# iamarkaj/AwesomeSLAM

Measured on AMD Instinct MI355X. Metric: EKF/UKF filter-steps/s @ N_landmarks, higher is better.
Workload: dtype f32

## Files before the change

awesomeslam_amd/core.py:

```python
import ctypes
import os
import subprocess

import numpy as np

_CSRC = os.path.join(os.path.dirname(os.path.abspath(__file__)), "csrc")
_CORE = os.path.join(_CSRC, "libaslam_core.so")
_NODE = os.path.join(_CSRC, "libaslam_node.so")

EKF, UKF = 0, 1
F64, F32 = 0, 1
FILTERS = {"ekf": EKF, "ukf": UKF}

ST_GROWTH_REFUSED, ST_WAIT_OVERFLOW, ST_NOT_PD, ST_OBS_OVERFLOW, ST_INTERNAL = 1, 2, 4, 8, 16
CFG_UKF_LARGE = 1

CORE_SYMBOLS = (
    "aslam_create", "aslam_destroy", "aslam_reset", "aslam_last_error", "aslam_abi_version", "aslam_set_state",
    "aslam_grow", "aslam_ekf_step", "aslam_ukf_step", "aslam_ekf_step_batch", "aslam_ukf_step_batch", "aslam_set_trace", "aslam_replay", "aslam_get_dim",
    "aslam_get_state", "aslam_get_A", "aslam_get_landmarks", "aslam_get_wait", "aslam_get_status",
    "aslam_get_layout", "aslam_kernel_info", "aslam_get_launch_info",
    "aslam_replay_stats", "aslam_innovation_enable", "aslam_get_innovation",
    "aslam_params_default", "aslam_set_params", "aslam_get_params",
    "aslam_remove_landmarks", "aslam_select_beyond",
    "aslam_get_sightings", "aslam_select_stale",
    "aslam_sighted_update_enable", "aslam_get_sighted", "aslam_ekf_step_sighted", "aslam_ekf_step_batch_sighted",
)
NODE_SYMBOLS = (
    "aslam_node_create", "aslam_node_create_at", "aslam_node_destroy", "aslam_node_error", "aslam_node_sensor", "aslam_node_odom",
    "aslam_node_odom_now", "aslam_node_dim", "aslam_node_get", "aslam_node_wait", "aslam_node_core",
    "aslam_host_narrow_odom", "aslam_node_enable_innovation", "aslam_node_innovation",
    "aslam_node_set_params", "aslam_node_get_params", "aslam_node_remove_landmarks",
    "aslam_node_get_sightings", "aslam_node_remove_stale", "aslam_node_set_sighted_only",
)
TRACE_FILE_SYMBOLS = (
    "aslam_trace_file_open", "aslam_trace_file_close", "aslam_trace_file_error", "aslam_trace_file_dims",
    "aslam_trace_file_view", "aslam_trace_file_raw", "aslam_trace_file_write",
)


class AslamError(RuntimeError):
    pass


class Config(ctypes.Structure):
    _fields_ = [(k, ctypes.c_int32) for k in
                ("filter", "dtype", "max_landmark_count", "batch", "max_obs", "max_wait", "device", "flags")]


class TraceView(ctypes.Structure):
    _fields_ = [("T", ctypes.c_int64), ("max_obs", ctypes.c_int32), ("is_device", ctypes.c_int32),
                ("pose", ctypes.c_void_p), ("yaw", ctypes.c_void_p), ("twist", ctypes.c_void_p),
                ("dt", ctypes.c_void_p), ("obs_new", ctypes.c_void_p), ("n_obs", ctypes.c_void_p),
                ("obs", ctypes.c_void_p)]
# ... 80 lines not shown
                          "(there is no CPU fallback for the filter core)")
        import torch

        L = ctypes.CDLL(_CORE)
        vp, ci, cf, cd = ctypes.c_void_p, ctypes.c_int, ctypes.c_float, ctypes.c_double
        pd, pf, pi, pu = (ctypes.POINTER(t) for t in (ctypes.c_double, ctypes.c_float, ctypes.c_int, ctypes.c_uint32))
        L.aslam_last_error.restype = ctypes.c_char_p
        L.aslam_create.argtypes = [ctypes.POINTER(Config), ctypes.POINTER(vp)]
        L.aslam_destroy.argtypes = [vp]
        L.aslam_reset.argtypes = [vp]
        L.aslam_set_state.argtypes = [vp, ci, ci, pd, pd, pd]
        L.aslam_grow.argtypes = [vp, ci, ci, pd, pd]
        L.aslam_ekf_step.argtypes = [vp, ci, cf, cf, cf, pd, cd, cd, pd, vp]
        L.aslam_ukf_step.argtypes = [vp, ci, cf, cf, cf, pd, pd, vp]
        L.aslam_ekf_step_batch.argtypes = [vp, pf, pf, pf, pd, ci, pd, pd, pd, ci, vp]
        L.aslam_ukf_step_batch.argtypes = [vp, pf, pf, pf, pd, ci, pd, ci, vp]
        L.aslam_set_trace.argtypes = [vp, ctypes.POINTER(TraceView)]
        L.aslam_replay.argtypes = [vp, ctypes.c_int64, ctypes.c_int64, vp, vp, vp]
        L.aslam_replay_stats.argtypes = [vp, ctypes.c_int64, ctypes.c_int64, vp, vp, vp, vp, vp, vp]
        L.aslam_innovation_enable.argtypes = [vp, ci]
        L.aslam_get_innovation.argtypes = [vp, ci, pd, pd]
        L.aslam_params_default.argtypes = [ctypes.POINTER(Params)]
        L.aslam_set_params.argtypes = [vp, ci, ctypes.POINTER(Params)]
        L.aslam_get_params.argtypes = [vp, ci, ctypes.POINTER(Params)]
        L.aslam_get_dim.argtypes = [vp, ci, pi]
        L.aslam_get_state.argtypes = [vp, ci, pd, pd, pd]
        L.aslam_get_A.argtypes = [vp, ci, pd, pd]
        L.aslam_get_landmarks.argtypes = [vp, ci, pd, pd, pi]
        L.aslam_get_wait.argtypes = [vp, ci, pf, pf, pu, ci, pi]
        L.aslam_get_status.argtypes = [vp, ci, pu]
        L.aslam_get_layout.argtypes = [vp, pi, ctypes.POINTER(ctypes.c_int64)]
        L.aslam_kernel_info.argtypes = [vp, ctypes.c_char_p, ci, pi, pi, pi]
        L.aslam_get_launch_info.argtypes = [vp, pi, pi, pi]
        L.aslam_remove_landmarks.argtypes = [vp, vp, ci, ci, vp]
        L.aslam_select_beyond.argtypes = [vp, pd, vp, ci, vp]
        L.aslam_get_sightings.argtypes = [vp, ci, pu, pu, ci, pi, pu]
        L.aslam_select_stale.argtypes = [vp, pu, vp, ci, vp]
        pb = ctypes.POINTER(ctypes.c_uint8)
        L.aslam_sighted_update_enable.argtypes = [vp, ci]
        L.aslam_get_sighted.argtypes = [vp, ci, pb, ci, pi]
        L.aslam_ekf_step_sighted.argtypes = [vp, ci, cf, cf, cf, pd, pb, cd, cd, pd, vp]
        L.aslam_ekf_step_batch_sighted.argtypes = [vp, pf, pf, pf, pd, ci, pb, ci, pd, pd, pd, ci, vp]
        p32, p64 = ctypes.POINTER(ctypes.c_int32), ctypes.POINTER(ctypes.c_int64)
        L.aslam_snapshot_record_bytes.restype = ctypes.c_int64
        L.aslam_snapshot_record_bytes.argtypes = [ci, ci, ci]
        L.aslam_snapshot_check.argtypes = [vp, ctypes.c_int64, p32, p32]
        L.aslam_snapshot.argtypes = [vp, p32, ci, vp, ctypes.c_int64, ci, p64, vp]
        L.aslam_restore.argtypes = [vp, p32, p32, ci, vp, ctypes.c_int64, ci, vp]
        _core = L
    return _core


def node_lib():
    global _node
    if _node is None:
        if not os.path.exists(_NODE):
            raise OSError(f"{_NODE} is missing: run __graft_entry__.build()")
        core_lib()
        L = ctypes.CDLL(_NODE)
        vp, ci = ctypes.c_void_p, ctypes.c_int
        pd, pf, pu = (ctypes.POINTER(t) for t in (ctypes.c_double, ctypes.c_float, ctypes.c_uint32))
        L.aslam_node_create.restype = vp
        L.aslam_node_create.argtypes = [ci, ci, ci]
        L.aslam_node_create_at.restype = vp
        L.aslam_node_create_at.argtypes = [ci, ci, ci, ctypes.c_double]
        L.aslam_node_destroy.argtypes = [vp]
# ... 422 lines not shown
        return (before - after) // 2

    def replay_forget(self, t0, nsteps, period, max_age, poses_ptr=None, dims_ptr=None, stream=None):
        t0, nsteps, period = int(t0), int(nsteps), int(period)
        if period < 1:
            raise ValueError("period must be at least 1")
        mask, ld = self._device_mask()
        dims, done = [], 0
        while done < nsteps:
            k = min(period, nsteps - done)
            self.replay(t0 + done, k, None if poses_ptr is None else poses_ptr + 8 * 3 * self.batch * done,
                        None if dims_ptr is None else dims_ptr + 4 * self.batch * done, stream)
            self.select_stale(max_age, mask.data_ptr(), ld, stream)
            dims.append(self.remove_landmarks(mask, stream=stream))
            done += k
        return np.array(dims, np.int64).reshape(len(dims), self.batch)

    def layout(self):
        npad, nbytes = ctypes.c_int(), ctypes.c_int64()
        _chk(core_lib().aslam_get_layout(self._h, ctypes.byref(npad), ctypes.byref(nbytes)))
        return npad.value, nbytes.value

    def kernel_info(self):
        name = ctypes.create_string_buffer(192)
        g, b, l = ctypes.c_int(), ctypes.c_int(), ctypes.c_int()
        _chk(core_lib().aslam_kernel_info(self._h, name, 192, ctypes.byref(g), ctypes.byref(b), ctypes.byref(l)))
        return {"name": name.value.decode(), "grid": g.value, "block": b.value, "lds_bytes": l.value}

    def launch_info(self):
        g, r, l = ctypes.c_int(), ctypes.c_int(), ctypes.c_int()
        _chk(core_lib().aslam_get_launch_info(self._h, ctypes.byref(g), ctypes.byref(r), ctypes.byref(l)))
        return {"stream_groups": g.value, "chol_resident": bool(r.value), "launches_per_callback": l.value}


class Node:

    def __init__(self, filter="ekf", max_landmark_count=30, device=0, now_init=0.0):
        h = node_lib().aslam_node_create_at(FILTERS[filter], int(max_landmark_count), int(device), float(now_init))
        if not h:
            raise AslamError(node_lib().aslam_node_error().decode())
        self._h = ctypes.c_void_p(h)

    def close(self):
        if getattr(self, "_h", None):
            node_lib().aslam_node_destroy(self._h)
            self._h = None

    __del__ = close

    def sensor_msg(self, xs, ys):
        xs = np.ascontiguousarray(xs, np.float64)
        ys = np.ascontiguousarray(ys, np.float64)
        node_lib().aslam_node_sensor(self._h, len(xs), _ptr(xs, ctypes.c_double), _ptr(ys, ctypes.c_double))

    def odom_msg(self, msg8, dt):
        m = np.ascontiguousarray(msg8, np.float64)
        rc = node_lib().aslam_node_odom(self._h, _ptr(m, ctypes.c_double), float(np.float32(dt)))
        if rc < 0:
            raise AslamError(node_lib().aslam_node_error().decode())
        return rc

    def odom_msg_now(self, msg8, now):
        m = np.ascontiguousarray(msg8, np.float64)
        rc = node_lib().aslam_node_odom_now(self._h, _ptr(m, ctypes.c_double), float(now))
        if rc < 0:
            raise AslamError(node_lib().aslam_node_error().decode())
# ... 82 lines not shown
```

awesomeslam_amd/csrc/aslam_core.hip:

```cpp
#include "../../include/aslam_core.h"
#include "../../include/aslam_scan.h"
#include "../../include/aslam_snapshot.h"

#include <hip/hip_runtime.h>

#include <cmath>
#include <cstdio>
#include <cstring>
#include <cstdlib>
#include <algorithm>
#include <mutex>
#include <string>
#include <type_traits>
#include <vector>

#include "ekf_small.h"
#include "ekf_large.h"
#include "ekf_large_launch.h"
#include "scan_front.h"
#include "snapshot.h"
#include "prune.h"
#if ASLAM_HAVE_UKF
#include "ukf_small.h"
#include "ukf_large.h"
// ... 1616 lines not shown
                hipLaunchKernelGGL(scan_landmarks_kernel, dim3((unsigned)count), dim3(64), 0, st, d_in, tab, tab + SCAN_BEAMS, count, max_out, d_r,
                                   d_b, d_n, d_s);
                e = hipGetLastError();
        }
        if (e == hipSuccess)
                e = hipMemcpyAsync(range_out, d_r, n * max_out * sizeof(float), hipMemcpyDeviceToHost, st);
        if (e == hipSuccess)
                e = hipMemcpyAsync(bearing_out, d_b, n * max_out * sizeof(float), hipMemcpyDeviceToHost, st);
        if (e == hipSuccess)
                e = hipMemcpyAsync(n_out, d_n, n * sizeof(int32_t), hipMemcpyDeviceToHost, st);
        if (e == hipSuccess)
                e = hipMemcpyAsync(status_out, d_s, n * sizeof(uint32_t), hipMemcpyDeviceToHost, st);
        if (e == hipSuccess)
                e = hipStreamSynchronize(st);
        cleanup();
        if (e != hipSuccess)
                return fail(ASLAM_ERR_HIP, std::string("aslam_scan_landmarks: ") + hipGetErrorString(e));
        return ASLAM_OK;
}

int aslam_get_launch_info(aslam_ctx *c, int *stream_groups, int *chol_resident, int *launches_per_callback)
{
        if (!c)
                return fail(ASLAM_ERR_ARG, "null context");
        if (stream_groups)
                *stream_groups = c->large ? c->lh.last_groups : 0;
        if (chol_resident)
                *chol_resident = c->large && c->lh.last_resident;
        if (launches_per_callback)
                *launches_per_callback = c->large ? c->lh.last_launches : 1;
        return ASLAM_OK;
}

int aslam_kernel_info(aslam_ctx *c, char *name, int name_cap, int *grid, int *block, int *lds_bytes)
{
        if (!c)
                return fail(ASLAM_ERR_ARG, "null context");
        char buf[192];
        size_t lds = 0;
        if (c->large)
        {
                const LargePlan plan = large_plan(c->cfg.dtype == ASLAM_F32, c->NP, c->cfg.batch, c->cfg.batch, c->lh.knobs);
#if ASLAM_HAVE_UKF
                if (c->cfg.filter == ASLAM_UKF)
                        std::snprintf(buf, sizeof(buf), "ukf_large_wabt + large_update_panel<double> + large_syrk<double> (%d-launch chain per callback, 1 stream)",
                                      ukf_large_plan(c->NP).launches);
                else
#endif
                if (plan.chain == LargeChain::F32_RESIDENT)
                        std::snprintf(buf, sizeof(buf), "%s + %s + large_syrk_bf16x3%s (%d-launch chain per callback, %d stream groups)",
                                      plan.chol16 ? "large_chol_bf16" : "large_chol_resident", plan.trsm16 ? "large_trsm_bf16" : "large_trsm_pipe<17>",
                                      plan.border ? " + border" : "", plan.launches, c->lh.knobs.groups);
                else if (plan.chain == LargeChain::F32_RIGHT)
                        std::snprintf(buf, sizeof(buf), "large_right_step + large_syrk_bf16x3 (%d-launch chain per callback: one right-looking launch per block column)", plan.launches);
                else if (plan.chain == LargeChain::F32_LEFT)
                        std::snprintf(buf, sizeof(buf), "large_trsm_pipe<17> + large_syrk_bf16x3 (%d-launch chain per callback: multi-workgroup Cholesky)", plan.launches);
                else
                        std::snprintf(buf, sizeof(buf), "large_update_panel<double> (%d-launch chain per callback, %d stream groups)", plan.launches, c->lh.knobs.groups);
                lds = LargeLds::bytes(c->NP);
                if (c->sighted_on && c->cfg.filter == ASLAM_EKF)
                {
                        const std::string with = std::string("large_build_GS<T,sighted> + ") + buf;
                        std::snprintf(buf, sizeof(buf), "%s", with.c_str());
                }
        }
        else if (c->cfg.filter == ASLAM_EKF)
// ... 27 lines not shown
```

awesomeslam_amd/csrc/ekf_large.h:

```cpp
#pragma once

#include <type_traits>

#include "small_common.h"

namespace aslam
{
constexpr int LB = 64;
constexpr int LARGE_OBS_CAP = 1024;
constexpr int LARGE_WAIT_CAP = 2048;
constexpr int LARGE_NP_MAX = 1088;
constexpr int LARGE_NB_MAX = LARGE_NP_MAX / LB;

template <typename T> struct LargeView
{
        int NP;
        double *P;
        T *G;
        T *S;
        double *Hc;
        double *Y;
        T *Linv;
        T *Vw;
        unsigned short *Lpl;
        int xrows;
        int border;
};

typedef float f4 __attribute__((ext_vector_type(4)));
template <typename T> struct Mfma;
template <> struct Mfma<double>
{
        typedef d4 acc_t;
        static __device__ __forceinline__ acc_t zero()
        {
                return (acc_t){0.0, 0.0, 0.0, 0.0};
        }
        static __device__ __forceinline__ acc_t mma(double a, double b, acc_t c)
        {
                return __builtin_amdgcn_mfma_f64_16x16x4f64(a, b, c, 0, 0, 0);
        }
        static __device__ __forceinline__ int row(int lane, int r)
        {
                return (lane >> 4) + 4 * r;
        }
};
template <> struct Mfma<float>
{
        typedef f4 acc_t;
        static __device__ __forceinline__ acc_t zero()
        {
                return (acc_t){0.f, 0.f, 0.f, 0.f};
        }
        static __device__ __forceinline__ acc_t mma(float a, float b, acc_t c)
        {
                return __builtin_amdgcn_mfma_f32_16x16x4f32(a, b, c, 0, 0, 0);
        }
        static __device__ __forceinline__ int row(int lane, int r)
        {
// ... 31 lines not shown
        const size_t np = (size_t)v.NP;
        f(v.P, np * np, false);
        f(v.G, np * np, true);
        f(v.S, np * np, true);
        f(v.Hc, (np / 2) * 4, false);
        f(v.Y, np, false);
        f(v.Linv, (size_t)LARGE_NB_MAX * LB * LB, false);
        f(v.Lpl, LPlanes::per_filter(v.NP), false);
        f(v.Vw, np * np, true);
}

__host__ __device__ __forceinline__ int lplane_pos(int c)
{
        return 32 * (c >> 5) + 8 * ((c >> 2) & 3) + 4 * ((c >> 4) & 1) + (c & 3);
}

__host__ __device__ __forceinline__ int large_blocks(int n, int xrows = 1)
{
        return (n + xrows + LB - 1) / LB;
}

struct LargeBorder
{
        int t;
        int nbc;
};
__host__ __device__ __forceinline__ LargeBorder large_border(int n, int enabled)
{
        const int n0 = n & ~(LB - 1), t = n - n0;
        const bool on = enabled && n0 >= LB && (t == 1 || t == 3);
        return {on ? t : 0, on ? n0 / LB : large_blocks(n)};
}
constexpr int BORDER_MAX = 3;
constexpr int BORDER_SAVE = 8, BORDER_SAVE_ROWS = 4;
__host__ __device__ __forceinline__ bool border_spare(const LargeBorder &bd, int n, int row, int col)
{
        return bd.t && row > n && row <= n + bd.t && (col < LB * bd.nbc || (col >= LB * bd.nbc + BORDER_SAVE && col < LB * bd.nbc + BORDER_SAVE + BORDER_SAVE_ROWS));
}

struct LargeLds
{
        static __host__ __device__ size_t bytes(int NP)
        {
                size_t o = 0;
                o += 8 * (size_t)NP * 2;
                o += 4 * (size_t)LARGE_OBS_CAP * 6;
                o += 4 * (size_t)LARGE_WAIT_CAP * 5;
                o += 4 * (size_t)(NP / 2);
                o += 4 * (size_t)LARGE_OBS_CAP * 4 * 2;
                o += 4 * (size_t)NP;
                o = (o + 15) & ~(size_t)15;
                return o + sizeof(SmallShared);
        }
        static __device__ __forceinline__ SmallLds carve(unsigned char *smem, int NP)
        {
                SmallLds L;
                unsigned char *p = smem;
                L.Lt = nullptr;
                L.Dinv = nullptr;
                L.sY = nullptr;
                L.sU = nullptr;
                L.sH = nullptr;
                L.sTv = nullptr;
                L.sX = reinterpret_cast<double *>(p);
                p += 8 * (size_t)NP;
                L.sZ = reinterpret_cast<double *>(p);
// ... 887 lines not shown
constexpr int XU_WAVES = ASLAM_XU_WAVES;
constexpr int XU_THREADS = 64 * XU_WAVES;
constexpr int XU_WG_ROWS = XU_WAVES * XU_ROWS;
typedef double xu_d2 __attribute__((ext_vector_type(2)));
constexpr int XU_STAGE_THREADS = 256;
static_assert(XU_WAVES >= 4 && XU_WAVES <= 16, "large_x_update_rows: 4 staging waves at least, 1024 threads at most");

template <bool RUNNING>
__global__ __launch_bounds__(256, 3) void large_syrk_bf16x3(DevView d, LargeView<float> lv, int nfilters, const int *skipped)
{
        constexpr int TB = 128, KC = 32;
        constexpr int LDB = KC;
        typedef __bf16 bf8 __attribute__((ext_vector_type(8)));
        typedef unsigned u4 __attribute__((ext_vector_type(4)));
        typedef unsigned u2 __attribute__((ext_vector_type(2)));
        __shared__ __attribute__((aligned(16))) unsigned short As[3][TB * LDB];
        __shared__ __attribute__((aligned(16))) unsigned short Bs[3][TB * LDB];
        const int ntile = (lv.NP + TB - 1) / TB, nlow = ntile * (ntile + 1) / 2;
        const int slot = blockIdx.x >> 3;
        const int b = (slot / nlow) * 8 + (blockIdx.x & 7);
        if (b >= nfilters || skipped[b])
                return;
        const int n = d.n[b], NP = lv.NP;
        const int na = large_blocks(n) * LB;
        const int tl = slot % nlow;
        int rt = (int)((sqrtf(8.0f * (float)tl + 1.0f) - 1.0f) * 0.5f);
        while ((rt + 1) * (rt + 2) / 2 <= tl)
                ++rt;
        while (rt * (rt + 1) / 2 > tl)
                --rt;
        const int jt = tl - rt * (rt + 1) / 2;
        if (rt * TB >= n)
                return;
        const int tid = threadIdx.x, wave = tid >> 6, lane = tid & 63, li = lane & 15, lg = lane >> 4;
        const int wr = (wave >> 1) * 64, wc = (wave & 1) * 64;
        const float *G = lv.G + (size_t)b * NP * NP;
        double *P = lv.P + (size_t)b * NP * NP;
        constexpr int LPR = KC / 4, RPP = 256 / LPR, NPASS = TB / RPP;
        const int lrow = tid / LPR, lc0 = (tid % LPR) * 4;
        const float *Ap[NPASS], *Bp[NPASS];
#pragma unroll
        for (int q = 0; q < NPASS; ++q)
        {
                Ap[q] = G + (size_t)min(rt * TB + lrow + RPP * q, na - 1) * NP + lc0;
                Bp[q] = G + (size_t)min(jt * TB + lrow + RPP * q, na - 1) * NP + lc0;
        }
        f4 acc[4][4];
#pragma unroll
        for (int u = 0; u < 4; ++u)
#pragma unroll
                for (int v = 0; v < 4; ++v)
                        acc[u][v] = (f4){0.f, 0.f, 0.f, 0.f};
        f4 ta[NPASS], tb[NPASS];
        auto fetch = [&](int kc) {
#pragma unroll
                for (int q = 0; q < NPASS; ++q)
                {
                        ta[q] = *reinterpret_cast<const f4 *>(Ap[q] + kc);
                        tb[q] = *reinterpret_cast<const f4 *>(Bp[q] + kc);
                }
        };
        typedef float f2 __attribute__((ext_vector_type(2)));
        typedef __bf16 bf2 __attribute__((ext_vector_type(2)));
        auto stash = [&](unsigned short (&S)[3][TB * LDB], int off, const f4 &x) {
                unsigned pk[3][2];
#pragma unroll
                for (int e = 0; e < 2; ++e)
                {
                        const f2 v = {x[2 * e], x[2 * e + 1]};
                        const bf2 h = __builtin_convertvector(v, bf2);
                        const f2 r1 = v - __builtin_convertvector(h, f2);
                        const bf2 m = __builtin_convertvector(r1, bf2);
                        const f2 r2 = r1 - __builtin_convertvector(m, f2);
                        const bf2 l = __builtin_convertvector(r2, bf2);
                        pk[0][e] = __builtin_bit_cast(unsigned, h), pk[1][e] = __builtin_bit_cast(unsigned, m), pk[2][e] = __builtin_bit_cast(unsigned, l);
                }
#pragma unroll
                for (int p = 0; p < 3; ++p)
                        *reinterpret_cast<u2 *>(&S[p][off]) = (u2){pk[p][0], pk[p][1]};
        };
        const bool idle = (rt == jt && wc > wr);
        const bool diagq = (rt == jt && wc == wr);
        const int nu = idle ? 0 : __builtin_amdgcn_readfirstlane(max(0, min(4, (n - (rt * TB + wr) + 15) >> 4)));
        const int nv = idle ? 0 : __builtin_amdgcn_readfirstlane(max(0, min(4, (n - (jt * TB + wc) + 15) >> 4)));
        const bool full = !RUNNING && nu == 4 && nv == 4 && !diagq;
        const int kend = min(na, (n + KC - 1) / KC * KC);
        const int a_off = (wr + li) * LDB + 8 * (lg ^ (li >> 2)), b_off = (wc + li) * LDB + 8 * (lg ^ (li >> 2));
        const int s_off = lrow * LDB + 8 * ((lc0 >> 3) ^ ((lrow & 15) >> 2)) + (lc0 & 4);
        fetch(0);
        for (int kc = 0; kc < kend; kc += KC)
        {
#pragma unroll
                for (int q = 0; q < NPASS; ++q)
                {
                        stash(As, s_off + RPP * q * LDB, ta[q]);
                        stash(Bs, s_off + RPP * q * LDB, tb[q]);
                }
                __syncthreads();
                if (kc + KC < kend)
                        fetch(kc + KC);
#define ASLAM_MM(t, bb, aa, c) t = __builtin_amdgcn_mfma_f32_16x16x32_bf16(__builtin_bit_cast(bf8, bb), __builtin_bit_cast(bf8, aa), c, 0, 0, 0)
                if (full)
                {
#pragma unroll
                        for (int vh = 0; vh < 4; vh += 2)
                        {
                                u4 bq[2][3];
#pragma unroll
                                for (int v = 0; v < 2; ++v)
#pragma unroll
                                        for (int p = 0; p < 3; ++p)
                                                bq[v][p] = *reinterpret_cast<const u4 *>(&Bs[p][b_off + 16 * (vh + v) * LDB]);
                                f4 pa = {0.f, 0.f, 0.f, 0.f}, pb = {0.f, 0.f, 0.f, 0.f};
#pragma unroll
                                for (int u = 0; u < 4; ++u)
                                {
                                        u4 ap[3];
#pragma unroll
                                        for (int p = 0; p < 3; ++p)
                                                ap[p] = *reinterpret_cast<const u4 *>(&As[p][a_off + 16 * u * LDB]);
                                        f4 ta, tb;
                                        ASLAM_MM(ta, bq[0][0], ap[2], ((f4){0.f, 0.f, 0.f, 0.f}));
                                        ASLAM_MM(tb, bq[1][0], ap[2], ((f4){0.f, 0.f, 0.f, 0.f}));
                                        ASLAM_MM(ta, bq[0][1], ap[1], ta);
                                        ASLAM_MM(tb, bq[1][1], ap[1], tb);
                                        ASLAM_MM(ta, bq[0][2], ap[0], ta);
                                        ASLAM_MM(tb, bq[1][2], ap[0], tb);
                                        if (u > 0)
                                        {
                                                acc[u - 1][vh] += pa;
                                                acc[u - 1][vh + 1] += pb;
                                        }
                                        ASLAM_MM(ta, bq[0][0], ap[1], ta);
                                        ASLAM_MM(tb, bq[1][0], ap[1], tb);
                                        ASLAM_MM(ta, bq[0][1], ap[0], ta);
                                        ASLAM_MM(tb, bq[1][1], ap[0], tb);
                                        ASLAM_MM(ta, bq[0][0], ap[0], ta);
                                        ASLAM_MM(tb, bq[1][0], ap[0], tb);
                                        pa = ta, pb = tb;
                                        __builtin_amdgcn_sched_barrier(0);
                                }
                                acc[3][vh] += pa;
                                acc[3][vh + 1] += pb;
                        }
                }
                else
                {
#pragma unroll
                        for (int vh = 0; vh < 4; vh += 2)
                        {
                                u4 bq[2][3];
#pragma unroll
                                for (int v = 0; v < 2; ++v)
#pragma unroll
                                        for (int p = 0; p < 3; ++p)
                                                bq[v][p] = *reinterpret_cast<const u4 *>(&Bs[p][b_off + 16 * (vh + v) * LDB]);
#pragma unroll
                                for (int u = 0; u < 4; ++u)
                                        if (u < nu)
                                        {
                                                u4 ap[3];
#pragma unroll
                                                for (int p = 0; p < 3; ++p)
                                                        ap[p] = *reinterpret_cast<const u4 *>(&As[p][a_off + 16 * u * LDB]);
#pragma unroll
                                                for (int v = 0; v < 2; ++v)
                                                        if (vh + v < nv && !(diagq && vh + v > u))
                                                        {
                                                                f4 tmp;
                                                                if constexpr (RUNNING)
                                                                {
                                                                        ASLAM_MM(tmp, bq[v][0], ap[2], acc[u][vh + v]);
                                                                        ASLAM_MM(tmp, bq[v][1], ap[1], tmp);
                                                                        ASLAM_MM(tmp, bq[v][2], ap[0], tmp);
                                                                        ASLAM_MM(tmp, bq[v][0], ap[1], tmp);
                                                                        ASLAM_MM(tmp, bq[v][1], ap[0], tmp);
                                                                        ASLAM_MM(tmp, bq[v][0], ap[0], tmp);
                                                                        acc[u][vh + v] = tmp;
                                                                        continue;
                                                                }
                                                                ASLAM_MM(tmp, bq[v][0], ap[2], ((f4){0.f, 0.f, 0.f, 0.f}));
                                                                ASLAM_MM(tmp, bq[v][1], ap[1], tmp);
                                                                ASLAM_MM(tmp, bq[v][2], ap[0], tmp);
                                                                ASLAM_MM(tmp, bq[v][0], ap[1], tmp);
                                                                ASLAM_MM(tmp, bq[v][1], ap[0], tmp);
                                                                ASLAM_MM(tmp, bq[v][0], ap[0], tmp);
                                                                acc[u][vh + v] += tmp;
                                                        }
                                        }
                        }
                }
#undef ASLAM_MM
                __syncthreads();
        }
        if (idle)
                return;
        const bool mirror = (jt < rt || wc < wr);
        const bool posecols_lane = (jt == 0 && wc == 0 && lg == 0);
        {
                typedef double d2 __attribute__((ext_vector_type(2)));
#pragma unroll
                for (int u = 0; u < 4; ++u)
#pragma unroll
                        for (int v = 0; v < 4; ++v)
                        {
                                const int row = rt * TB + wr + 16 * u + li;
                                const int col0 = jt * TB + wc + 16 * v + 4 * lg;
                                if (row >= n || col0 >= n || (diagq && v > u))
                                        continue;
                                const bool posecols = posecols_lane && v == 0;
                                if ((diagq && v == u) || posecols)
                                {
#pragma unroll
                                        for (int r = 0; r < 4; ++r)
                                                if (col0 + r < row && !(posecols && r < 3) && col0 + r < n)
                                                {
                                                        double *pe = P + (size_t)row * NP + col0 + r;
                                                        const double pn = *pe - (double)acc[u][v][r];
                                                        *pe = pn;
                                                        P[(size_t)(col0 + r) * NP + row] = pn;
                                                }
                                        continue;
                                }
                                double *pp = P + (size_t)row * NP + col0;
                                double nv4[4];
                                if (col0 + 3 < n)
                                {
                                        const d2 o0 = *reinterpret_cast<const d2 *>(pp), o1 = *reinterpret_cast<const d2 *>(pp + 2);
                                        nv4[0] = o0[0] - (double)acc[u][v][0], nv4[1] = o0[1] - (double)acc[u][v][1];
                                        nv4[2] = o1[0] - (double)acc[u][v][2], nv4[3] = o1[1] - (double)acc[u][v][3];
                                        *reinterpret_cast<d2 *>(pp) = (d2){nv4[0], nv4[1]};
                                        *reinterpret_cast<d2 *>(pp + 2) = (d2){nv4[2], nv4[3]};
                                }
                                else
                                {
#pragma unroll
                                        for (int r = 0; r < 4; ++r)
                                                if (col0 + r < n)
                                                {
                                                        nv4[r] = pp[r] - (double)acc[u][v][r];
                                                        pp[r] = nv4[r];
                                                }
                                }
                                if (mirror || diagq)
                                {
#pragma unroll
                                        for (int r = 0; r < 4; ++r)
                                                if (col0 + r < n)
                                                        P[(size_t)(col0 + r) * NP + row] = nv4[r];
                                }
                        }
        }
}

template <typename T, int MODE>
__global__ __launch_bounds__(256) void large_x_update(DevView d, LargeView<T> lv, int s, int nsteps, double *poses_out,
                                                      int32_t *dims_out, const int *skipped)
{
        const int b = blockIdx.y;
        if (skipped[b])
                return;
        const int n = d.n[b], NP = lv.NP;
        const int a = blockIdx.x * 4 + (threadIdx.x >> 6), lane = threadIdx.x & 63;
        if (a >= n)
                return;
        const T *vrow = lv.G + ((size_t)b * NP + a) * NP;
        const T *q = lv.G + ((size_t)b * NP + n) * NP;
        double acc = 0.0;
        typedef T vec_t __attribute__((ext_vector_type(16 / sizeof(T))));
        constexpr int VW = 16 / sizeof(T);
        for (int j = VW * lane; j < n; j += 64 * VW)
        {
                const vec_t v = *reinterpret_cast<const vec_t *>(vrow + j), w = *reinterpret_cast<const vec_t *>(q + j);
#pragma unroll
                for (int e = 0; e < VW; ++e)
                        acc = fma((double)v[e], (double)w[e], acc);
        }
        acc = wave_sum_dpp(acc);
        if (lane == 63)
        {
                const double xa = d.X[(size_t)b * NP + a] + acc;
                d.X[(size_t)b * NP + a] = xa;
                if (MODE == MODE_REPLAY)
                {
                        if (a < 3 && poses_out)
// ... 430 lines not shown
```

awesomeslam_amd/csrc/ekf_large_launch.h:

```cpp
#pragma once

#include <hip/hip_runtime.h>

#include <algorithm>
#include <cstdlib>

#include "ekf_large.h"
#include "aslam_large16.h"

namespace aslam
{
constexpr int LARGE_GROUPS_MAX = 8;
constexpr int CHOL_RESIDENT_MIN_BATCH = 32;

struct LargeKnobs
{
        int groups = 3;
        int chol_resident = -1;
        int right_step = 1;
        int bf16_pipe = 3;
        int keep_l32 = 0;
        int gs_tiles = 0;
        int border = 1;
        int syrk_running = 0;
};

inline LargeKnobs large_knobs_from_env()
{
        LargeKnobs k;
        auto flag = [](const char *name, int &v) { if (const char *e = std::getenv(name)) v = std::atoi(e) != 0; };
        if (const char *e = std::getenv("ASLAM_LARGE_GROUPS"))
                k.groups = std::max(1, std::min(LARGE_GROUPS_MAX, std::atoi(e)));
        if (const char *e = std::getenv("ASLAM_BF16_PIPE"))
                k.bf16_pipe = std::atoi(e) & 3;
        flag("ASLAM_CHOL_RESIDENT", k.chol_resident);
        flag("ASLAM_RIGHT_STEP", k.right_step);
        flag("ASLAM_KEEP_L32", k.keep_l32);
        flag("ASLAM_GS_TILES", k.gs_tiles);
        flag("ASLAM_SYRK_RUNNING", k.syrk_running);
        flag("ASLAM_BORDER", k.border);
        return k;
}

enum class LargeChain
{
        F64_LEFT,
        F32_RESIDENT,
        F32_RIGHT,
        F32_LEFT
};

struct LargePlan
{
        LargeChain chain;
        bool chol16, trsm16;
        bool border;
        bool chol_f32out;
        bool gs_tiles, syrk_running;
        int launches;
        bool need_Lpl, need_Vw;
};

inline LargePlan large_plan(bool f32, int NP, int batch, int filters, const LargeKnobs &k)
{
        const int NB = NP / LB;
        auto resident = [&k](int nf) { return k.chol_resident >= 0 ? k.chol_resident != 0 : nf >= CHOL_RESIDENT_MIN_BATCH; };
        LargePlan p = {};
        p.gs_tiles = k.gs_tiles != 0;
        p.syrk_running = k.syrk_running != 0;
        p.need_Lpl = f32 && k.bf16_pipe != 0;
        p.need_Vw = f32 && k.right_step && !resident(batch);
        if (!f32)
                p.chain = LargeChain::F64_LEFT, p.launches = 4 + 2 * NB;
        else if (resident(filters))
        {
                p.chain = LargeChain::F32_RESIDENT, p.launches = 6;
                p.chol16 = (k.bf16_pipe & 2) != 0;
                p.trsm16 = (k.bf16_pipe & 1) != 0;
                p.chol_f32out = !p.trsm16 || k.keep_l32;
                p.border = p.chol16 && p.trsm16 && !k.keep_l32 && k.border != 0;
        }
        else if (p.need_Vw)
                p.chain = LargeChain::F32_RIGHT, p.launches = 5 + NB;
        else
                p.chain = LargeChain::F32_LEFT, p.launches = 4 + 2 * NB;
        return p;
}

struct LargeHost
{
        LargeKnobs knobs;
        hipStream_t aux[LARGE_GROUPS_MAX - 1] = {};
        hipEvent_t ev_fork = nullptr, ev_join[LARGE_GROUPS_MAX - 1] = {};
        int last_groups = 0;
        int last_launches = 0;
        bool last_resident = false;
        bool sighted = false;
};

struct LaunchSlice
{
        int first, count;
        StepArgs sa;
};
template <int MODE> LaunchSlice launch_slice(StepArgs sa, int B)
{
        if (MODE != MODE_STEP || sa.traj < 0)
                return {0, B, sa};
        const int first = sa.traj;
        sa.traj = 0;
        return {first, 1, sa};
}

struct ShiftBy
{
        size_t b;
        template <typename T> void operator()(T *&p, size_t per, bool) const
        {
                if (p)
                        p += b * per;
        }
};

template <typename V, typename... NP> V shifted(V v, size_t b, NP... np)
{
        static_assert(!std::is_same<V, DevView>::value && !std::is_same<V, StatsView>::value, "shifted_dev / shifted_stats");
        for_each_array(v, np..., ShiftBy{b});
        return v;
}
// ... 117 lines not shown
                        hipLaunchKernelGGL((large_x_update_rows<MODE>), dim3((NP + XU_WG_ROWS - 1) / XU_WG_ROWS, gb), dim3(XU_THREADS), 0, g.st, g.dv, vv, s, nsteps,
                                           g.poses, g.dims, g.skip);
                };
                if (plan.border)
                        x_update();
                if (plan.syrk_running)
                        hipLaunchKernelGGL((large_syrk_bf16x3<true>), syrk_grid, dim3(256), 0, g.st, g.dv, vv, gb, g.skip);
                else
                        hipLaunchKernelGGL((large_syrk_bf16x3<false>), syrk_grid, dim3(256), 0, g.st, g.dv, vv, gb, g.skip);
                if (!plan.border)
                        x_update();
                if (g.sv.any())
                        hipLaunchKernelGGL(large_stats<T>, dim3(gb), dim3(256), 0, g.st, g.dv, vv, s, nsteps, g.sv, g.skip);
        }
}

template <int MODE, typename T>
hipError_t launch_large(LargeHost &h, const DevView &dv, const LargeView<T> &lv, int *skipped, int64_t t0, int nsteps, double *poses, int32_t *dims,
                        StepArgs sa, hipStream_t st, StatsView sv = {})
{
        const size_t lds = LargeLds::bytes(dv.NP);
        if (hipError_t e = h.sighted ? hipFuncSetAttribute(reinterpret_cast<const void *>(large_frontend_kernel<T, MODE, true>), hipFuncAttributeMaxDynamicSharedMemorySize, (int)lds)
                                     : hipFuncSetAttribute(reinterpret_cast<const void *>(large_frontend_kernel<T, MODE>), hipFuncAttributeMaxDynamicSharedMemorySize, (int)lds))
                return e;
        const LaunchSlice sl = launch_slice<MODE>(sa, dv.B);
        const int first = sl.first, Bz = sl.count;
        const LargePlan plan = large_plan(sizeof(T) == 4, dv.NP, dv.B, Bz, h.knobs);
        const bool split = Bz >= std::max(32, 8 * h.knobs.groups);
        const int NG = split ? h.knobs.groups : 1;
        const int per = split ? ((Bz + NG - 1) / NG + 7) & ~7 : Bz;
        LargeGroup<T> g[LARGE_GROUPS_MAX];
        h.last_launches = plan.launches + (sv.any() ? 1 : 0);
        h.last_resident = plan.chain == LargeChain::F32_RESIDENT;
        h.last_groups = 0;
        for (int q = 0; q < NG; ++q)
        {
                const int o = std::min(q * per, Bz);
                const size_t b0 = (size_t)(first + o);
                g[q] = {shifted_dev(dv, b0, MODE == MODE_REPLAY), shifted(lv, b0), skipped + b0, poses, dims, std::min(per, Bz - o), q == 0 ? st : h.aux[q - 1], shifted_stats(sv, b0, nsteps)};
                g[q].v.border = plan.border;
                if (MODE == MODE_REPLAY && poses)
                        g[q].poses += b0 * (size_t)nsteps * 3;
                if (MODE == MODE_REPLAY && dims)
                        g[q].dims += b0 * (size_t)nsteps;
                h.last_groups += g[q].nb > 0;
        }
        hipError_t e = split ? hipEventRecord(h.ev_fork, st) : hipSuccess;
        for (int q = 1; q < NG && e == hipSuccess; ++q)
                e = hipStreamWaitEvent(h.aux[q - 1], h.ev_fork, 0);
        if (e != hipSuccess)
                return e;
        for (int s = 0; s < nsteps; ++s)
                for (int q = 0; q < NG; ++q)
                        if (g[q].nb > 0)
                                launch_large_chain<T, MODE>(plan, g[q], lds, t0, s, nsteps, sl.sa, h.sighted);
        for (int q = 1; q < NG && e == hipSuccess; ++q)
                if ((e = hipEventRecord(h.ev_join[q - 1], h.aux[q - 1])) == hipSuccess)
                        e = hipStreamWaitEvent(st, h.ev_join[q - 1], 0);
        return e != hipSuccess ? e : hipGetLastError();
}
}
```

awesomeslam_amd/csrc/ukf_large_launch.h:

```cpp
#pragma once

#include "ekf_large_launch.h"
#include "ukf_large.h"

namespace aslam
{
struct UkfLargePlan
{
        int NB;
        int frontend;
        int chol_p;
        int sigma;
        int products;
        int solve;
        int update;
        int launches;
};

inline UkfLargePlan ukf_large_plan(int NP)
{
        UkfLargePlan p = {};
        p.NB = NP / LB;
        p.frontend = 1;
        p.chol_p = 2 * p.NB - 1;
        p.sigma = 2;
        p.products = 3;
        p.solve = 2 * p.NB;
        p.update = 3;
        p.launches = p.frontend + p.chol_p + p.sigma + p.products + p.solve + p.update;
        return p;
}

template <int MODE>
hipError_t launch_ukf_large(LargeHost &h, const DevView &dv0, const LargeView<double> &lv0, const UkfLargeView &uv0, int *skipped0, int64_t t0, int nsteps,
                            double *poses, int32_t *dims, StepArgs sa, hipStream_t st, StatsView sv0 = {})
{
        const int NP = dv0.NP;
        const size_t lds = LargeLds::bytes(NP);
        if (hipError_t e = hipFuncSetAttribute(reinterpret_cast<const void *>(ukf_large_frontend_kernel<MODE>), hipFuncAttributeMaxDynamicSharedMemorySize, (int)lds))
                return e;
        const LaunchSlice sl = launch_slice<MODE>(sa, dv0.B);
        const size_t first = (size_t)sl.first;
        const int gb = sl.count;
        const DevView dv = shifted_dev(dv0, first, MODE == MODE_REPLAY);
        const LargeView<double> lv = shifted(lv0, first);
        const UkfLargeView uv = shifted(uv0, first, NP);
        int *skip = skipped0 + first;
        const StatsView sv = shifted_stats(sv0, first, nsteps);
        const UkfLargePlan plan = ukf_large_plan(NP);
        const int NB = plan.NB;
        const int ntile = (NP + 127) / 128;
        const int fgroups = (gb + 7) / 8;
        h.last_launches = plan.launches + (sv.any() ? 1 : 0);
        h.last_resident = false;
        h.last_groups = 1;
        for (int s = 0; s < nsteps; ++s)
        {
                int count = 0;
                hipLaunchKernelGGL((ukf_large_frontend_kernel<MODE>), dim3(gb), dim3(SMALL_WG), lds, st, dv, lv, uv, t0 + s, s, nsteps, poses, dims, sl.sa, skip);
                count += plan.frontend;
                count += launch_left_looking(dv, lv, NB, gb, skip, st, 1, false);
                hipLaunchKernelGGL(ukf_large_sigma_pose, dim3(gb), dim3(256), 0, st, dv, lv, uv, skip);
                hipLaunchKernelGGL(ukf_large_points, dim3(NP / 2, gb), dim3(256), 0, st, dv, lv, uv, skip);
                count += plan.sigma;
                for (int mode : {WABT_P, WABT_S, WABT_TC})
                {
                        hipLaunchKernelGGL(ukf_large_wabt, dim3(8 * ukf_wabt_tiles(NP, mode) * fgroups), dim3(256), 0, st, dv, lv, uv, mode, gb, skip);
                        ++count;
                }
                count += launch_left_looking(dv, lv, NB, gb, skip, st, 0, true);
                hipLaunchKernelGGL((ukf_large_gain<MODE>), dim3((NP + 3) / 4, gb), dim3(256), 0, st, dv, lv, uv, s, nsteps, poses, dims, skip);
                hipLaunchKernelGGL(large_syrk<double>, dim3(8 * (ntile * (ntile + 1) / 2) * fgroups), dim3(256), 0, st, dv, lv, gb, skip);
                hipLaunchKernelGGL(ukf_large_rank1, dim3((NP + 3) / 4, gb), dim3(256), 0, st, dv, lv, uv, skip);
                count += plan.update;
                if (count != plan.launches)
                        return hipErrorAssert;
                if (sv.any())
                        hipLaunchKernelGGL(large_stats<double>, dim3(gb), dim3(256), 0, st, dv, lv, s, nsteps, sv, skip);
        }
        return hipGetLastError();
}
}
```

include/aslam_core.h:

```cpp
#ifndef ASLAM_CORE_H
#define ASLAM_CORE_H

#include <stdint.h>

#ifdef __cplusplus
extern "C" {
#endif

#define ASLAM_ABI_VERSION 1

enum
{
        ASLAM_OK = 0,
        ASLAM_ERR_ARG = -1,
        ASLAM_ERR_HIP = -2,
        ASLAM_ERR_UNSUPPORTED = -3,
        ASLAM_ERR_STATE = -4
};

enum
{
        ASLAM_EKF = 0,
        ASLAM_UKF = 1
};
// ... 89 lines not shown
                         const double *a00, const double *a10, double *X_out, int ldx, void *stream);
int aslam_ukf_step_batch(aslam_ctx *ctx, const float *vx, const float *az, const float *dt, const double *Z, int ldz,
                         double *X_out, int ldx, void *stream);
int aslam_ekf_step_sighted(aslam_ctx *ctx, int traj, float vx, float az, float dt, const double *Z, const uint8_t *sighted, double a00,
                           double a10, double *X_out, void *stream);
int aslam_ekf_step_batch_sighted(aslam_ctx *ctx, const float *vx, const float *az, const float *dt, const double *Z, int ldz,
                                 const uint8_t *sighted, int ld, const double *a00, const double *a10, double *X_out, int ldx, void *stream);

int aslam_set_trace(aslam_ctx *ctx, const aslam_trace *trace);
int aslam_replay(aslam_ctx *ctx, int64_t t0, int64_t nsteps, double *poses_out, int32_t *dims_out, void *stream);
int aslam_replay_stats(aslam_ctx *ctx, int64_t t0, int64_t nsteps, double *poses_out, int32_t *dims_out, double *nis_out,
                       double *logdet_out, double *pose_cov_out, void *stream);
int aslam_innovation_enable(aslam_ctx *ctx, int on);
int aslam_get_innovation(aslam_ctx *ctx, int traj, double *nis, double *logdet);

int aslam_sighted_update_enable(aslam_ctx *ctx, int on);
int aslam_get_sighted(aslam_ctx *ctx, int traj, uint8_t *sighted, int cap, int *n_landmarks);

int aslam_remove_landmarks(aslam_ctx *ctx, const uint8_t *mask, int ld, int is_device, void *stream);
int aslam_select_beyond(aslam_ctx *ctx, const double *max_range, uint8_t *mask_dev, int ld, void *stream);

int aslam_get_sightings(aslam_ctx *ctx, int traj, uint32_t *last_seen, uint32_t *hits, int cap, int *n_landmarks, uint32_t *clock);
int aslam_select_stale(aslam_ctx *ctx, const uint32_t *max_age, uint8_t *mask_dev, int ld, void *stream);

int aslam_get_dim(aslam_ctx *ctx, int traj, int *n);
int aslam_get_state(aslam_ctx *ctx, int traj, double *X, double *Z, double *P);
int aslam_get_A(aslam_ctx *ctx, int traj, double *a00, double *a10);
int aslam_get_landmarks(aslam_ctx *ctx, int traj, double *x, double *y, int *n_landmarks);
int aslam_get_wait(aslam_ctx *ctx, int traj, float *range, float *bearing, uint32_t *count, int cap, int *size);
int aslam_get_status(aslam_ctx *ctx, int traj, uint32_t *status_bits);
int aslam_get_layout(aslam_ctx *ctx, int *padded_dim, int64_t *hbm_bytes);
int aslam_kernel_info(aslam_ctx *ctx, char *name, int name_cap, int *grid, int *block, int *lds_bytes);
int aslam_get_launch_info(aslam_ctx *ctx, int *stream_groups, int *chol_resident, int *launches_per_callback);

#ifdef __cplusplus
}
#endif
#endif
```

Before: 39890.

## Fold thin SYRK tail row-tile into idle waves of preceding tiles

When the last 128-row tile of the covariance SYRK update holds only a few rows (at most 16), its off-diagonal tile blocks are skipped. Otherwise-idle waves in the tiles above compute those thin rows instead, using bf16x3 split MFMA against the shared B tile and writing the mirrored P entries. This removes mostly-empty workgroups and wasted MFMA work for N just past a multiple of 128. In exchange it adds register pressure and extra global loads in the idle-wave path. The behaviour is controlled by an env flag that defaults to on for the f32 non-running path, and a query API is added.

```diff
diff --git a/awesomeslam_amd/core.py b/awesomeslam_amd/core.py
--- a/awesomeslam_amd/core.py
+++ b/awesomeslam_amd/core.py
@@ -19,7 +19,7 @@
     "aslam_create", "aslam_destroy", "aslam_reset", "aslam_last_error", "aslam_abi_version", "aslam_set_state",
     "aslam_grow", "aslam_ekf_step", "aslam_ukf_step", "aslam_ekf_step_batch", "aslam_ukf_step_batch", "aslam_set_trace", "aslam_replay", "aslam_get_dim",
     "aslam_get_state", "aslam_get_A", "aslam_get_landmarks", "aslam_get_wait", "aslam_get_status",
-    "aslam_get_layout", "aslam_kernel_info", "aslam_get_launch_info",
+    "aslam_get_layout", "aslam_kernel_info", "aslam_get_launch_info", "aslam_get_syrk_tail",
     "aslam_replay_stats", "aslam_innovation_enable", "aslam_get_innovation",
     "aslam_params_default", "aslam_set_params", "aslam_get_params",
     "aslam_remove_landmarks", "aslam_select_beyond",
@@ -166,6 +166,7 @@
         L.aslam_get_layout.argtypes = [vp, pi, ctypes.POINTER(ctypes.c_int64)]
         L.aslam_kernel_info.argtypes = [vp, ctypes.c_char_p, ci, pi, pi, pi]
         L.aslam_get_launch_info.argtypes = [vp, pi, pi, pi]
+        L.aslam_get_syrk_tail.argtypes = [vp, pi]
         L.aslam_remove_landmarks.argtypes = [vp, vp, ci, ci, vp]
         L.aslam_select_beyond.argtypes = [vp, pd, vp, ci, vp]
         L.aslam_get_sightings.argtypes = [vp, ci, pu, pu, ci, pi, pu]
@@ -654,6 +655,11 @@
         _chk(core_lib().aslam_get_launch_info(self._h, ctypes.byref(g), ctypes.byref(r), ctypes.byref(l)))
         return {"stream_groups": g.value, "chol_resident": bool(r.value), "launches_per_callback": l.value}
 
+    def syrk_tail(self):
+        on = ctypes.c_int()
+        _chk(core_lib().aslam_get_syrk_tail(self._h, ctypes.byref(on)))
+        return bool(on.value)
+
 
 class Node:
 
diff --git a/awesomeslam_amd/csrc/aslam_core.hip b/awesomeslam_amd/csrc/aslam_core.hip
--- a/awesomeslam_amd/csrc/aslam_core.hip
+++ b/awesomeslam_amd/csrc/aslam_core.hip
@@ -1672,6 +1672,14 @@
         return ASLAM_OK;
 }
 
+int aslam_get_syrk_tail(aslam_ctx *c, int *on)
+{
+        if (!c || !on)
+                return fail(ASLAM_ERR_ARG, "null argument");
+        *on = c->large && c->lh.last_syrk_tail;
+        return ASLAM_OK;
+}
+
 int aslam_kernel_info(aslam_ctx *c, char *name, int name_cap, int *grid, int *block, int *lds_bytes)
 {
         if (!c)
diff --git a/awesomeslam_amd/csrc/ekf_large.h b/awesomeslam_amd/csrc/ekf_large.h
--- a/awesomeslam_amd/csrc/ekf_large.h
+++ b/awesomeslam_amd/csrc/ekf_large.h
@@ -25,6 +25,7 @@
         unsigned short *Lpl;
         int xrows;
         int border;
+        int syrk_tail;
 };
 
 typedef float f4 __attribute__((ext_vector_type(4)));
@@ -122,6 +123,17 @@
         return {on ? t : 0, on ? n0 / LB : large_blocks(n)};
 }
 constexpr int BORDER_MAX = 3;
+
+struct SyrkTail
+{
+        int rl;
+        int rows;
+};
+__host__ __device__ __forceinline__ SyrkTail large_syrk_tail(int n, int enabled)
+{
+        const int rl = (n - 1) / 128, t = n - 128 * rl;
+        return {rl, enabled && rl >= 1 && t <= 16 ? t : 0};
+}
 constexpr int BORDER_SAVE = 8, BORDER_SAVE_ROWS = 4;
 __host__ __device__ __forceinline__ bool border_spare(const LargeBorder &bd, int n, int row, int col)
 {
@@ -1075,6 +1087,9 @@
         const int jt = tl - rt * (rt + 1) / 2;
         if (rt * TB >= n)
                 return;
+        const SyrkTail tail = large_syrk_tail(n, !RUNNING && lv.syrk_tail);
+        if (tail.rows && rt == tail.rl && jt < rt)
+                return;
         const int tid = threadIdx.x, wave = tid >> 6, lane = tid & 63, li = lane & 15, lg = lane >> 4;
         const int wr = (wave >> 1) * 64, wc = (wave & 1) * 64;
         const float *G = lv.G + (size_t)b * NP * NP;
@@ -1130,7 +1145,18 @@
         const int kend = min(na, (n + KC - 1) / KC * KC);
         const int a_off = (wr + li) * LDB + 8 * (lg ^ (li >> 2)), b_off = (wc + li) * LDB + 8 * (lg ^ (li >> 2));
         const int s_off = lrow * LDB + 8 * ((lc0 >> 3) ^ ((lrow & 15) >> 2)) + (lc0 & 4);
+        const bool tailw = idle && tail.rows && rt < tail.rl;
+        f4 &tp0 = acc[3][0], &tp1 = acc[3][1];
+        if (tailw)
+                acc[3][2][0] = __builtin_bit_cast(float, 4u * (unsigned)(min(tail.rl * TB + li, na - 1) * NP + 8 * lg));
+        auto tail_fetch = [&](int kc) {
+                const char *row = reinterpret_cast<const char *>(G + kc) + __builtin_bit_cast(unsigned, acc[3][2][0]);
+                tp0 = *reinterpret_cast<const f4 *>(row);
+                tp1 = *reinterpret_cast<const f4 *>(row + 16);
+        };
         fetch(0);
+        if (tailw)
+                tail_fetch(0);
         for (int kc = 0; kc < kend; kc += KC)
         {
 #pragma unroll
@@ -1187,6 +1213,32 @@
                                 acc[3][vh + 1] += pb;
                         }
                 }
+                else if (tailw)
+                {
+                        u2x h0, m0, l0, h1, m1, l1;
+                        split_bf16x3(tp0, h0, m0, l0);
+                        split_bf16x3(tp1, h1, m1, l1);
+                        const u4 ap[3] = {(u4){h0[0], h0[1], h1[0], h1[1]}, (u4){m0[0], m0[1], m1[0], m1[1]}, (u4){l0[0], l0[1], l1[0], l1[1]}};
+                        if (kc + KC < kend)
+                                tail_fetch(kc + KC);
+#pragma unroll
+                        for (int v = 0; v < 8; ++v)
+                        {
+                                u4 bq[3];
+#pragma unroll
+                                for (int p = 0; p < 3; ++p)
+                                        bq[p] = *reinterpret_cast<const u4 *>(&Bs[p][b_off + (16 * v - wc) * LDB]);
+                                f4 tmp;
+                                ASLAM_MM(tmp, bq[0], ap[2], ((f4){0.f, 0.f, 0.f, 0.f}));
+                                ASLAM_MM(tmp, bq[1], ap[1], tmp);
+                                ASLAM_MM(tmp, bq[2], ap[0], tmp);
+                                ASLAM_MM(tmp, bq[0], ap[1], tmp);
+                                ASLAM_MM(tmp, bq[1], ap[0], tmp);
+                                ASLAM_MM(tmp, bq[0], ap[0], tmp);
+                                acc[v >> 2][v & 3] += tmp;
+                                __builtin_amdgcn_sched_barrier(0);
+                        }
+                }
                 else
                 {
 #pragma unroll
@@ -1236,64 +1288,73 @@
 #undef ASLAM_MM
                 __syncthreads();
         }
-        if (idle)
+        if (idle && !tailw)
                 return;
         const bool mirror = (jt < rt || wc < wr);
+        typedef double d2 __attribute__((ext_vector_type(2)));
+        auto update4 = [&](int row, int col0, const f4 &a, bool diag16, bool posecols, bool mir) {
+                if (diag16 || posecols)
+                {
+#pragma unroll
+                        for (int r = 0; r < 4; ++r)
+                                if (col0 + r < row && !(posecols && r < 3) && col0 + r < n)
+                                {
+                                        double *pe = P + (size_t)row * NP + col0 + r;
+                                        const double pn = *pe - (double)a[r];
+                                        *pe = pn;
+                                        P[(size_t)(col0 + r) * NP + row] = pn;
+                                }
+                        return;
+                }
+                double *pp = P + (size_t)row * NP + col0;
+                double nv4[4];
+                if (col0 + 3 < n)
+                {
+                        const d2 o0 = *reinterpret_cast<const d2 *>(pp), o1 = *reinterpret_cast<const d2 *>(pp + 2);
+                        nv4[0] = o0[0] - (double)a[0], nv4[1] = o0[1] - (double)a[1];
+                        nv4[2] = o1[0] - (double)a[2], nv4[3] = o1[1] - (double)a[3];
+                        *reinterpret_cast<d2 *>(pp) = (d2){nv4[0], nv4[1]};
+                        *reinterpret_cast<d2 *>(pp + 2) = (d2){nv4[2], nv4[3]};
+                }
+                else
+                {
+#pragma unroll
+                        for (int r = 0; r < 4; ++r)
+                                if (col0 + r < n)
+                                {
+                                        nv4[r] = pp[r] - (double)a[r];
+                                        pp[r] = nv4[r];
+                                }
+                }
+                if (mir)
+                {
+#pragma unroll
+                        for (int r = 0; r < 4; ++r)
+                                if (col0 + r < n)
+                                        P[(size_t)(col0 + r) * NP + row] = nv4[r];
+                }
+        };
+        if (tailw)
+        {
+                const int row = tail.rl * TB + li;
+                if (row < n)
+#pragma unroll
+                        for (int v = 0; v < 8; ++v)
+                                update4(row, jt * TB + 16 * v + 4 * lg, acc[v >> 2][v & 3], false, jt == 0 && lg == 0 && v == 0, true);
+                return;
+        }
         const bool posecols_lane = (jt == 0 && wc == 0 && lg == 0);
-        {
-                typedef double d2 __attribute__((ext_vector_type(2)));
-#pragma unroll
-                for (int u = 0; u < 4; ++u)
-#pragma unroll
-                        for (int v = 0; v < 4; ++v)
-                        {
-                                const int row = rt * TB + wr + 16 * u + li;
-                                const int col0 = jt * TB + wc + 16 * v + 4 * lg;
-                                if (row >= n || col0 >= n || (diagq && v > u))
-                                        continue;
-                                const bool posecols = posecols_lane && v == 0;
-                                if ((diagq && v == u) || posecols)
-                                {
-#pragma unroll
-                                        for (int r = 0; r < 4; ++r)
-                                                if (col0 + r < row && !(posecols && r < 3) && col0 + r < n)
-                                                {
-                                                        double *pe = P + (size_t)row * NP + col0 + r;
-                                                        const double pn = *pe - (double)acc[u][v][r];
-                                                        *pe = pn;
-                                                        P[(size_t)(col0 + r) * NP + row] = pn;
-                                                }
-                                        continue;
-                                }
-                                double *pp = P + (size_t)row * NP + col0;
-                                double nv4[4];
-                                if (col0 + 3 < n)
-                                {
-                                        const d2 o0 = *reinterpret_cast<const d2 *>(pp), o1 = *reinterpret_cast<const d2 *>(pp + 2);
-                                        nv4[0] = o0[0] - (double)acc[u][v][0], nv4[1] = o0[1] - (double)acc[u][v][1];
-                                        nv4[2] = o1[0] - (double)acc[u][v][2], nv4[3] = o1[1] - (double)acc[u][v][3];
-                                        *reinterpret_cast<d2 *>(pp) = (d2){nv4[0], nv4[1]};
-                                        *reinterpret_cast<d2 *>(pp + 2) = (d2){nv4[2], nv4[3]};
-                                }
-                                else
-                                {
-#pragma unroll
-                                        for (int r = 0; r < 4; ++r)
-                                                if (col0 + r < n)
-                                                {
-                                                        nv4[r] = pp[r] - (double)acc[u][v][r];
-                                                        pp[r] = nv4[r];
-                                                }
-                                }
-                                if (mirror || diagq)
-                                {
-#pragma unroll
-                                        for (int r = 0; r < 4; ++r)
-                                                if (col0 + r < n)
-                                                        P[(size_t)(col0 + r) * NP + row] = nv4[r];
-                                }
-                        }
-        }
+#pragma unroll
+        for (int u = 0; u < 4; ++u)
+#pragma unroll
+                for (int v = 0; v < 4; ++v)
+                {
+                        const int row = rt * TB + wr + 16 * u + li;
+                        const int col0 = jt * TB + wc + 16 * v + 4 * lg;
+                        if (row >= n || col0 >= n || (diagq && v > u))
+                                continue;
+                        update4(row, col0, acc[u][v], diagq && v == u, posecols_lane && v == 0 , mirror || diagq);
+                }
 }
 
 template <typename T, int MODE>
diff --git a/awesomeslam_amd/csrc/ekf_large_launch.h b/awesomeslam_amd/csrc/ekf_large_launch.h
--- a/awesomeslam_amd/csrc/ekf_large_launch.h
+++ b/awesomeslam_amd/csrc/ekf_large_launch.h
@@ -22,6 +22,7 @@
         int keep_l32 = 0;
         int gs_tiles = 0;
         int border = 1;
+        int syrk_tail = 1;
         int syrk_running = 0;
 };
 
@@ -39,6 +40,7 @@
         flag("ASLAM_GS_TILES", k.gs_tiles);
         flag("ASLAM_SYRK_RUNNING", k.syrk_running);
         flag("ASLAM_BORDER", k.border);
+        flag("ASLAM_SYRK_TAIL", k.syrk_tail);
         return k;
 }
 
@@ -57,6 +59,7 @@
         bool border;
         bool chol_f32out;
         bool gs_tiles, syrk_running;
+        bool syrk_tail;
         int launches;
         bool need_Lpl, need_Vw;
 };
@@ -68,6 +71,7 @@
         LargePlan p = {};
         p.gs_tiles = k.gs_tiles != 0;
         p.syrk_running = k.syrk_running != 0;
+        p.syrk_tail = f32 && !p.syrk_running && k.syrk_tail != 0;
         p.need_Lpl = f32 && k.bf16_pipe != 0;
         p.need_Vw = f32 && k.right_step && !resident(batch);
         if (!f32)
@@ -95,6 +99,7 @@
         int last_groups = 0;
         int last_launches = 0;
         bool last_resident = false;
+        bool last_syrk_tail = false;
         bool sighted = false;
 };
 
@@ -278,6 +283,7 @@
         LargeGroup<T> g[LARGE_GROUPS_MAX];
         h.last_launches = plan.launches + (sv.any() ? 1 : 0);
         h.last_resident = plan.chain == LargeChain::F32_RESIDENT;
+        h.last_syrk_tail = plan.syrk_tail;
         h.last_groups = 0;
         for (int q = 0; q < NG; ++q)
         {
@@ -285,6 +291,7 @@
                 const size_t b0 = (size_t)(first + o);
                 g[q] = {shifted_dev(dv, b0, MODE == MODE_REPLAY), shifted(lv, b0), skipped + b0, poses, dims, std::min(per, Bz - o), q == 0 ? st : h.aux[q - 1], shifted_stats(sv, b0, nsteps)};
                 g[q].v.border = plan.border;
+                g[q].v.syrk_tail = plan.syrk_tail;
                 if (MODE == MODE_REPLAY && poses)
                         g[q].poses += b0 * (size_t)nsteps * 3;
                 if (MODE == MODE_REPLAY && dims)
diff --git a/awesomeslam_amd/csrc/ukf_large_launch.h b/awesomeslam_amd/csrc/ukf_large_launch.h
--- a/awesomeslam_amd/csrc/ukf_large_launch.h
+++ b/awesomeslam_amd/csrc/ukf_large_launch.h
@@ -53,6 +53,7 @@
         const int fgroups = (gb + 7) / 8;
         h.last_launches = plan.launches + (sv.any() ? 1 : 0);
         h.last_resident = false;
+        h.last_syrk_tail = false;
         h.last_groups = 1;
         for (int s = 0; s < nsteps; ++s)
         {
diff --git a/include/aslam_core.h b/include/aslam_core.h
--- a/include/aslam_core.h
+++ b/include/aslam_core.h
@@ -145,6 +145,7 @@
 int aslam_get_layout(aslam_ctx *ctx, int *padded_dim, int64_t *hbm_bytes);
 int aslam_kernel_info(aslam_ctx *ctx, char *name, int name_cap, int *grid, int *block, int *lds_bytes);
 int aslam_get_launch_info(aslam_ctx *ctx, int *stream_groups, int *chol_resident, int *launches_per_callback);
+int aslam_get_syrk_tail(aslam_ctx *ctx, int *on);
 
 #ifdef __cplusplus
 }
```

Result: faster. 40740 (median of 6 runs) (+2.1%).
